# SayanoAI/Comfy-RVC

Hardware: AMD Instinct MI355X
Metric: audio-sec/wall-sec (xRT), 40k_v2 end-to-end VC (higher is better)
Workload: dtype f32; 1 GPU; Full VC 40k_v2 (HuBERT -> RMVPE -> SynthesizerTrnMs768NSFsid), 30 s 16 kHz clips, 12 per GPU per step (3 in flight), vc_single host array in -> int16 host array out (BASELINE.json configs[2]); clips_in_flight_per_gpu=3, weights=procedural (comfy-rvc_amd/synthetic.py), noise=device generator, seeded per clip, parallelism=clip-per-GPU x1 (3 lanes each), one RCCL gather of the step's int16 waveforms

## Files before the change

### comfy-rvc_amd/_lib.py

```python
import ctypes as C
import os

_HERE = os.path.dirname(os.path.abspath(__file__))
LIB_PATH = os.environ.get("RVC_HIP_LIB") or os.path.join(_HERE, "csrc", "librvc_hip.so")


class RvcHipError(RuntimeError):
    pass


def _load():
    if not os.path.isfile(LIB_PATH):
        raise RvcHipError(
            f"{LIB_PATH} is missing: build it with `python -c 'import __graft_entry__ as g; g.build()'` "
            "(or `make -C comfy-rvc_amd/csrc`).  There is no CPU fallback.")
    return C.CDLL(LIB_PATH)


lib = _load()

c_void_p, c_int, c_int64, c_float, c_char_p = C.c_void_p, C.c_int, C.c_int64, C.c_float, C.c_char_p
P = C.POINTER


# ... 177 lines not shown
    "rvc_segment_energy": (c_int, [c_void_p, c_void_p, c_int64, c_int, c_void_p]),
    "rvc_spectrogram_batch": (c_int, [c_void_p, c_void_p, c_void_p, c_int64, c_void_p, c_int, c_int, c_int, c_float, c_int, c_void_p, c_int64]),
    "rvc_mel_filterbank_set": (c_int, [c_void_p, c_int, c_int, c_void_p, c_void_p, c_void_p]),
    "rvc_spec_to_mel_batch": (c_int, [c_void_p, c_void_p, c_void_p, c_int64, c_void_p, c_int, c_int, c_int, c_void_p, c_int64]),
    "rvc_spectrogram_batch_ms": (c_int, [c_void_p, c_void_p, c_void_p, c_int64, c_void_p, c_int, c_int, c_int, c_float, c_int, c_void_p, c_int64]),
    "rvc_mel_spectrogram_vjp": (c_int, [c_void_p, c_void_p, c_void_p, c_int64, c_void_p, c_int, c_int, c_int, c_float, c_int, c_int, c_void_p, c_int64,
                                        c_void_p]),
    "rvc_mel_spectrogram_vjp_launch_count": (c_int, []),
    "rvc_mel_loss_cotangents": (c_int, [c_void_p, c_int, P(c_void_p), P(c_void_p), P(c_int64), c_int, c_float, c_float, P(c_float), P(c_void_p)]),
    "rvc_multiscale_mel_loss": (c_int, [c_void_p, c_void_p, c_int, P(c_void_p), P(c_int64), P(c_int64), c_int, c_int64, P(C.c_int32), P(C.c_int32), c_int, c_int,
                                        c_void_p]),
    "rvc_hpss": (c_int, [c_void_p, c_void_p, c_int, c_int, c_int, c_void_p, c_void_p, c_int]),
    "rvc_hpss_l1": (c_int, [c_void_p, c_void_p, c_void_p, c_int, c_int, c_int, c_float, c_void_p]),
    "rvc_tsi_terms": (c_int, [c_void_p, c_void_p, c_void_p, c_int, c_int, c_int, c_float, c_void_p]),
    "rvc_op_gemm_split": (c_int, [c_void_p] * 7 + [c_int] * 4 + [c_float, c_int, c_float] + [c_int] * 5),
    "rvc_op_conv2d_split": (c_int, [c_void_p] * 7 + [c_int] * 9),
    "rvc_op_wn_in_gate_split": (c_int, [c_void_p] * 6 + [c_int] * 4),
    "rvc_op_gemm_split_qkv": (c_int, [c_void_p] * 6 + [c_int] * 4),
    "rvc_op_conv1d_s2_split": (c_int, [c_void_p] * 6 + [c_int] * 5),
    "rvc_op_conv1d_split": (c_int, [c_void_p] * 6 + [c_int] * 9),
    "rvc_op_conv1d": (c_int, [c_void_p, c_void_p, c_void_p, c_void_p, c_void_p, c_void_p] + [c_int] * 8 +
                      [c_int, c_float, c_int, c_float, c_int, c_float, c_int]),
    "rvc_op_conv_transpose1d": (c_int, [c_void_p, c_void_p, c_void_p, c_void_p, c_void_p] + [c_int] * 6 + [c_int, c_float, c_int]),
    "rvc_op_conv2d3x3": (c_int, [c_void_p, c_void_p, c_void_p, c_void_p, c_void_p, c_void_p] + [c_int] * 5),
    "rvc_op_conv_transpose2d": (c_int, [c_void_p, c_void_p, c_void_p, c_void_p, c_void_p] + [c_int] * 5),
    "rvc_op_gemm_tn": (c_int, [c_void_p, c_void_p, c_void_p, c_void_p] + [c_int] * 4),
    "rvc_conv1d_plan_create": (c_int, [c_void_p, c_void_p] + [c_int] * 7 + [P(c_void_p)]),
    "rvc_conv1d_plan_run": (c_int, [c_void_p, c_void_p, c_void_p, c_int, c_void_p, c_void_p, c_int, c_float, c_int, c_float]),
    "rvc_conv1d_plan_pair_run": (c_int, [c_void_p, c_void_p, c_void_p, c_void_p, c_int, c_void_p, c_float, c_int]),
    "rvc_conv1d_plan_resblock_run": (c_int, [P(c_void_p), c_void_p, c_void_p, c_int, c_void_p, c_float, c_int, P(c_int), c_void_p, c_void_p, c_void_p]),
    "rvc_conv1d_plan_pair_split_run": (c_int, [c_void_p, c_void_p, c_void_p, c_void_p, c_int, c_void_p, c_float, c_int]),
    "rvc_conv1d_plan_destroy": (c_int, [c_void_p]),
    "rvc_op_attention": (c_int, [c_void_p, c_void_p, c_void_p, c_void_p, c_void_p, c_void_p, c_int, c_int]),
    "rvc_op_attention_split": (c_int, [c_void_p] * 7 + [c_int, c_int]),
    "rvc_op_attention_split_rel": (c_int, [c_void_p] * 9 + [c_int, c_int, c_int]),
    "rvc_op_cbr2_small": (c_int, [c_void_p] * 7 + [c_int, c_int, c_int]),
    "rvc_op_layernorm_c_split": (c_int, [c_void_p] * 6 + [c_int, c_int]),
    "rvc_op_conv3_small": (c_int, [c_void_p] * 7 + [c_int] * 6),
    "rvc_op_gemm_split_swapped": (c_int, [c_void_p] * 4 + [c_int] * 5),
    "rvc_op_conv2d3x3_plus_1x1": (c_int, [c_void_p] * 7 + [c_int] * 6),
    "rvc_op_gemm_split_swapped_res": (c_int, [c_void_p] * 5 + [c_int] * 5),
    "rvc_op_attention_rel": (c_int, [c_void_p] * 8 + [c_int, c_int, c_void_p, c_void_p]),
    "rvc_op_layernorm_c": (c_int, [c_void_p] * 6 + [c_int, c_int]),
    "rvc_resample": (c_int, [c_void_p, c_void_p, c_int64, c_void_p, c_int, c_int, c_int, c_void_p, c_int64]),
    "rvc_set_conv_precision": (c_int, [c_int]),
    "rvc_set_pair_arithmetic": (c_int, [c_int]),
# ... 112 lines not shown
```

### comfy-rvc_amd/csrc/conv_kernels.h

```cpp
#pragma once
#include "rvc_internal.h"
#include <hip/hip_ext.h>

namespace rvc {

typedef float f32x16 __attribute__((ext_vector_type(16)));
typedef unsigned int u32x4 __attribute__((ext_vector_type(4)));

struct ConvArgsX : ConvArgs {
  long long ldW;
  int Wcols;
  int Wrows;
  int ksplit; float* partial; long long ldP;
  unsigned magRP, magPW;
  int ni; unsigned magNI;
  const unsigned char* Wx; int CoPx; int xbufs; int NC; int kreal; long long wxBatch;
  const unsigned char* Wx2; const float* bias1; int fuse_p2; float fuse_slope;
  const unsigned char* Xs; long long xsTp;
  unsigned char* Ys; long long ysTp; float ys_slope;
  int wbufs;
  int xcd_remap;
  int h2;
};

// ... 126 lines not shown
bool conv_x3g_plan(ConvPlan& p);
bool conv_x3pf_plan(ConvPlan& p);
bool conv_rbh_plan(ConvPlan& p);
bool conv_x3_pair_plan(const ConvLayer& c1, const ConvLayer& c2, const float* X, long long ldX, int T, long long Tplan, float* Y, long long ldY,
                       const ConvEpilogue& e2, int h2, ConvPlan& p);

struct Rb3Args {
  const float* X; long long ldX; float* Y; long long ldY;
  const unsigned char* W[6];
  const float* B[6];
  int CoPx;
  int T, halo, NO;
  float pre_slope, mid_slope, out_scale;
  const float* nsrc; const float* nw; const float* nb;
};
struct Rb3Plan {
  Rb3Args a; void (*launch)(const Rb3Args&, dim3, size_t, hipStream_t) = nullptr; dim3 grid; size_t lds = 0;
  int C = 0, k = 0, accumulate = 0;
};
bool conv_rb3_plan(const ConvLayer* const* c1, const ConvLayer* const* c2, const float* X, long long ldX, int T, long long Tplan, float* Y, long long ldY,
                   float pre_slope, float out_scale, int accumulate, int h2, const float* nsrc, const float* nw, const float* nb, Rb3Plan& p);
void conv_rb3_launch(const Rb3Plan& p, hipStream_t s);

}
```

### comfy-rvc_amd/csrc/conv_mfma.hip

```cpp
#include "conv_kernels.h"
#include "phase_timing.h"
#include <atomic>
#include <tuple>

#ifndef RVC_EPI_TWOPHASE
#define RVC_EPI_TWOPHASE 0
#endif

namespace rvc {

RVC_PHASE_TABLE_REGISTER;

constexpr int kWSlots = 32;
__host__ __device__ constexpr int x_slots(int BN, int MODE) {
  return MODE == 2 ? (BN >= 512 ? 26 : (BN >= 256 ? 18 : 14)) : (BN >= 512 ? 36 : (BN >= 256 ? 20 : (BN >= 128 ? 32 : 16)));
}

template <int WM, int WN, int AM, int AN, int MODE>
__global__ __launch_bounds__(256) void conv_mfma_kernel(const ConvArgsX p) {
  constexpr int BM = WM * AM * 32, BN = WN * AN * 32;
  constexpr int XS = x_slots(BN, MODE);
  extern __shared__ __attribute__((aligned(16))) float smem[];
  const int CK = p.CK, WROW = p.WROW;
  float* Xs = smem;
// ... 525 lines not shown
  L.nchunk = (Ci + L.CK - 1) / L.CK;
  L.wBatch = (long long)L.nchunk * L.ktaps * L.CK * L.CoP;
  std::vector<float> P((size_t)L.wBatch, 0.f);
  for (int r = 0; r < u; ++r)
    for (int co = 0; co < Co; ++co)
      for (int ci = 0; ci < Ci; ++ci)
        for (int j = 0; j < L.ktaps; ++j) {
          const int e = E2 - j;
          const int kk = e * u + r + pad;
          if (kk < 0 || kk >= k) continue;
          const int chunk = ci / L.CK, vcc = ci % L.CK;
          P[(((size_t)chunk * L.ktaps + j) * L.CK + vcc) * L.CoP + (size_t)co * u + r] = w[((size_t)ci * Co + co) * k + kk];
        }
  if ((g_precision == 2 || (g_precision == 1 && g_x3_default)) && Ci % 16 == 0 && L.Co >= 32) {
    std::vector<float> Weq((size_t)L.Co * Ci * L.ktaps, 0.f);
    for (int r = 0; r < u; ++r)
      for (int co = 0; co < Co; ++co)
        for (int ci = 0; ci < Ci; ++ci)
          for (int j = 0; j < L.ktaps; ++j) {
            const int kk = (E2 - j) * u + r + pad;
            if (kk >= 0 && kk < k) Weq[(((size_t)co * u + r) * Ci + ci) * L.ktaps + j] = w[((size_t)ci * Co + co) * k + kk];
          }
    pack_x3(L, Weq.data(), L.Co, Ci, L.ktaps);
  }
  L.k = k; L.pad = pad;
  L.dil = 1;
  L.conv_pad = E2;
  upload_layer(L, P, bias, Co);
}

void conv2d_kx_layer_init(ConvLayer& L, const float* w, const float* bias, int Co, int Ci, int KH, int KW, int PH, int PWL) {
  RVC_REQUIRE(Ci % 16 == 0 && KH >= 1 && KW >= 1 && PH >= 0 && PH < KH && PWL >= 0 && PWL < KW, "conv2d_kx: Ci must be a multiple of 16, padding inside the window");
  L.mode = 2; L.groups = 1; L.Ci = Ci; L.Co = Co; L.co_real = Co; L.CoP = (Co + 31) & ~31;
  L.k = KH * KW; L.stride = 1; L.dil = 1; L.pad = 0; L.tconv_u = 0; L.up2 = 0; L.ktaps = KH * KW;
  L.kh = KH; L.kw = KW; L.ph = PH; L.pwl = PWL;
  L.CK = 16; L.nchunk = Ci / 16; L.wBatch = 0;
  pack_x3(L, w, Co, Ci, KH * KW);
  L.bd_ = bias ? dev_upload(bias, Co) : nullptr;
}
void conv2d3x3_layer_init(ConvLayer& L, const float* w, const float* bias, int Co, int Ci) {
  L.mode = 2; L.groups = 1; L.Ci = Ci; L.Co = Co; L.co_real = Co; L.CoP = (Co + 31) & ~31;
  L.k = 3; L.stride = 1; L.dil = 1; L.pad = 1; L.tconv_u = 0; L.up2 = 0; L.ktaps = 9;
  L.CK = pick_ck(Ci, 9, 1);
  L.nchunk = (Ci + L.CK - 1) / L.CK;
  L.wBatch = (long long)L.nchunk * 9 * L.CK * L.CoP;
  std::vector<float> P((size_t)L.wBatch, 0.f);
// ... 132 lines not shown
  pe.armed = false;
  if (pe.launches == 1) {
    (void)hipEventDestroy(t.a); (void)hipEventDestroy(t.b);
    t.a = pe.ka; t.b = pe.kb;
  } else {
    (void)hipEventDestroy(pe.ka); (void)hipEventDestroy(pe.kb);
  }
  pe.ka = pe.kb = nullptr;
  ProfRec r{t.a, t.b, flops, cfg, bytes, 0, 0, 0, 0, 0, 0, 0, 1, fused, blocks, 0};
  if (a) { r.h2 = a->h2; r.Ci = a->Ci; r.Co = a->Co; r.k = a->kreal > 0 ? a->kreal : a->ktaps; r.dil = a->dil; r.stride = a->stride; r.Tout = a->Tout; r.Wd = a->Wd; r.ksplit = a->ksplit > 0 ? a->ksplit : 1; }
  std::lock_guard<std::mutex> lk(g_prof_mu);
  g_prof.push_back(r);
}
int conv_prof_dump_csv(const char* path) {
  std::lock_guard<std::mutex> lk(g_prof_mu);
  FILE* f = fopen(path, "w");
  if (!f) return -1;
  fprintf(f, "launch,kernel,tile,Ci,Co,k,dil,stride,Tout,Wd,fused_pair,ksplit,workgroups,us,alg_gflop,alg_mbytes,tflops,alg_gbps,mfma_per_product\n");
  int i = 0;
  for (auto& r : g_prof) {
    (void)hipEventSynchronize(r.b);
    float t = 0.f;
    if (hipEventElapsedTime(&t, r.a, r.b) != hipSuccess) continue;
    static const char* kX3Fam[8] = {"conv_x3_kernel", "conv_x3p_kernel", "conv_x3g_kernel", "conv_x3pf_kernel", "conv_x3s_kernel", "conv_rbh_kernel", "conv_x3q_kernel", "conv_rb3_kernel"};
    fprintf(f, "%d,%s,%s,%d,%d,%d,%d,%d,%d,%d,%d,%d,%lld,%.2f,%.4f,%.3f,%.2f,%.1f,%d\n", i++, r.cfg >= 14 ? kX3Fam[(r.fused >> 4) & 7] : "conv_mfma_kernel", kCfgNames[r.cfg],
            r.Ci, r.Co, r.k, r.dil, r.stride, r.Tout, r.Wd, r.fused & 15, r.ksplit, r.blocks, t * 1e3, r.flops / 1e9, r.bytes / 1e6,
            t > 0 ? r.flops / t / 1e9 : 0.0, t > 0 ? r.bytes / t / 1e6 : 0.0, r.cfg >= 14 ? (r.h2 ? 2 : 3) : 1);
  }
  fclose(f);
  return i;
}
double conv_alg_bytes(const ConvArgsX& a, int batch) {
  const double in = (double)a.Ci * (a.Wd > 0 ? (double)a.Tin * a.Wd : (double)a.Tin);
  const double out = (double)a.Co * a.Tout;
  const double w = (double)a.Co * a.Ci * (a.kreal > 0 ? a.kreal : a.ktaps);
  const bool r_is_x = a.R != nullptr && a.R == a.X;
  return 4.0 * (batch * (in + out * (1.0 + ((a.R && !r_is_x) ? 1.0 : 0.0) + (a.accumulate ? 1.0 : 0.0))) + w);
}
int conv_prof_collect_ex(double* out, double ridge_fp32, double ridge_x3) {
  std::lock_guard<std::mutex> lk(g_prof_mu);
  for (int i = 0; i < kProfCfgs * 8; ++i) out[i] = 0;
  for (auto& r : g_prof) {
    (void)hipEventSynchronize(r.b);
    float t = 0.f;
    if (hipEventElapsedTime(&t, r.a, r.b) != hipSuccess) continue;
    const double ridge = r.cfg >= 14 ? ridge_x3 : ridge_fp32;
    const int o = (r.bytes > 0 && r.flops / r.bytes < ridge) ? 4 : 0;
    double* q = out + r.cfg * 8 + o;
// ... 135 lines not shown
  if (e.tout_limit > 0 && e.tout_limit < Tout) { RVC_REQUIRE(L.tconv_u == 0, "tout_limit on a transposed conv"); Tout = e.tout_limit; }
  auto gemm_cols = [&](int tout) { return L.tconv_u > 0 ? (tout + L.tconv_u - 1) / L.tconv_u : tout; };
  a.Tout = gemm_cols(Tout);
  RVC_REQUIRE(e.plan_tin == 0 || (e.plan_tin >= Tin && !e.tout_limit), "plan_tin is the input length of the whole sequence this launch is a column window of");
  const long long Tplan = e.plan_tin > 0 ? gemm_cols(conv1d_out_len(L, e.plan_tin)) : a.Tout;
  if (L.tconv_u > 0) {
    a.pad = L.conv_pad;
    a.ostride = L.tconv_u; a.orows = L.co_real;
    RVC_REQUIRE(ldY == Tout, "interleaved ConvTranspose1d store needs a dense output (ldY == Tout)");
    RVC_REQUIRE(e.R == nullptr, "residual not supported on the interleaved store");
  } else {
    a.pad = L.pad; a.ostride = 1; a.orows = L.Co;
  }
  a.xBatch = (long long)L.Ci * ldX; a.wBatch = L.wBatch; a.yBatch = (long long)L.Co * ldY; a.rBatch = (long long)L.Co * e.ldR;
  a.bBatch = L.Co;
  const double flops = L.tconv_u > 0 ? 2.0 * Tin * L.Ci * L.co_real * L.k
                                     : 2.0 * L.groups * (double)L.Co * a.Tout * L.Ci * L.k;
  a.Wx = reinterpret_cast<const unsigned char*>(L.Wx_); a.CoPx = L.CoPx; a.wxBatch = L.wxBatch; a.kreal = L.tconv_u > 0 ? L.ktaps : L.k;
  if (e.h2) {
    RVC_REQUIRE(L.Wh_ && (e.xs_in || e.ys_out), "fp16x2 arithmetic is for the two halves of a split-resident ResBlock pair (conv1d_pair_h2_eligible)");
    a.Wx = reinterpret_cast<const unsigned char*>(L.Wh_); a.h2 = 1;
  }
  ConvPlan p;
  if (L.Wx_ && conv_x3_plan(a, L.groups, Tplan, p)) { p.flops = flops; conv_plan_launch(p, s); }
  else {
    RVC_REQUIRE(!e.xs_in && !e.ys_out, "split-resident tensors need the bf16x3 kernel (check conv1d_split_eligible first)");
    run_conv(a, 1, L.groups, Tplan, s, flops);
  }
  if (post) {
    RVC_REQUIRE(L.tconv_u == 0, "post-activation on a transposed conv");
    act_res_inplace(s, Y, e0.R, L.groups * L.Co, Tout, ldY, e0.ldR, e0.act, e0.act_slope, e0.act_before_res);
  }
}

bool conv1d_pair_h2_eligible(const ConvLayer& c1, const ConvLayer& c2, int Tin, int h2) {
  if (!h2 || !c1.Wh_ || !c2.Wh_) return false;
  return conv1d_split_eligible(c1, Tin, SPLIT_PRODUCER, 1) && conv1d_split_eligible(c2, Tin, SPLIT_CONSUMER, 1);
}

static bool plan_split_role(const ConvLayer& L, int Tin, SplitRole role, int h2, ConvPlan& p) {
  if (L.mode != 1 || !L.Wx_ || (h2 && !L.Wh_) || L.tconv_u || L.stride != 1 || L.groups != 1 || (L.Co & 31) || (L.Ci & 15)) return false;
  if (conv1d_out_len(L, Tin) != Tin || L.pad > kSplitMargin) return false;
  ConvArgsX a{};
  a.Ci = L.Ci; a.Co = L.Co; a.CoP = L.CoP; a.Tin = Tin; a.Wd = 0; a.ktaps = L.ktaps; a.dil = L.dil; a.stride = 1; a.pad = L.pad;
  a.Tout = conv1d_out_len(L, Tin); a.ostride = 1; a.orows = L.Co; a.ldX = Tin; a.ldY = a.Tout; a.ldR = a.Tout;
  a.Wx = reinterpret_cast<const unsigned char*>(L.Wx_); a.CoPx = L.CoPx; a.kreal = L.k; a.h2 = h2;
  if (role == SPLIT_CONSUMER) a.R = reinterpret_cast<const float*>(L.Wx_);
// ... 63 lines not shown
```

### comfy-rvc_amd/csrc/rvc_api.hip

```cpp
#include "models.h"
#include "conv_kernels.h"

namespace rvc {
static thread_local std::string g_err;
void set_error(const std::string& msg) { g_err = msg; }
}

using namespace rvc;

struct rvc_ctx { Ctx c; };
static std::mutex g_ctx_mu;
static std::map<int, int> g_ctx_count;
struct rvc_hubert { Hubert* m; rvc_ctx* ctx; };
struct rvc_rmvpe { Rmvpe* m; rvc_ctx* ctx; };
struct rvc_synth { Synth* m; rvc_ctx* ctx; };
struct rvc_conv1d_plan { OwnedConvLayer L; };

#define RVC_TRY try {
#define RVC_CATCH                                                            \
  return 0;                                                                  \
  }                                                                          \
  catch (const std::exception& e) { rvc::set_error(e.what()); return 1; }    \
  catch (...) { rvc::set_error("unknown error"); return 2; }

// ... 1290 lines not shown
  xs.alloc(ib); RVC_HIP_CHECK(hipMemsetAsync(xs.p, 0, ib, s));
  yp.alloc((size_t)Co * T);
  pad2d_split(s, x, (long long)H * W, Ci, H, W, nullptr, 0, xs.p, tp, g.margin);
  ConvEpilogue e; e.act = act; e.act_slope = 0.1f; e.act_before_res = act_before_res;
  if (res) { rp.alloc((size_t)Co * T); pad2d_split(s, res, (long long)H * W, Co, H, W, rp.p, T, nullptr, 0, 0); e.R = rp.p; e.ldR = T; }
  if (ysplit_f32) { ys.alloc(ob); RVC_HIP_CHECK(hipMemsetAsync(ys.p, 0, ob, s)); e.ys_out = ys.p; e.ys_tp = tp; }
  { X3sForceScope force(ksplit, am, an); conv_x3s_run(L, s, xs.p, tp, T, yp.p, T, e, &g); }
  unpad2d(s, yp.p, T, Co, H, W, y, (long long)H * W);
  if (ysplit_f32) {
    RVC_REQUIRE((Co & 15) == 0, "split output needs Co % 16 == 0");
    t.alloc((size_t)Co * T);
    split_image_to_f32(s, ys.p + (size_t)(g.margin - kSplitMargin) * 16, tp, Co, T, t.p, T);
    unpad2d(s, t.p, T, Co, H, W, ysplit_f32, (long long)H * W);
  }
  check_launch();
  RVC_HIP_CHECK(hipStreamSynchronize(s));
  RVC_CATCH
}
int rvc_op_conv_transpose1d(void* stream, const float* x, const float* w, const float* bias, float* y, int Ci, int Co, int Tin, int k, int u,
                            int pad, int pre_act, float pre_slope, int accumulate) {
  RVC_TRY
  OwnedConvLayer L;
  tconv1d_layer_init(L, w, bias, Ci, Co, k, u, pad);
  ConvEpilogue e; e.pre_act = pre_act; e.pre_slope = pre_slope; e.accumulate = accumulate;
  const int Tout = conv1d_out_len(L, Tin);
  conv1d_run(L, (hipStream_t)stream, x, Tin, Tin, y, Tout, e);
  check_launch();
  RVC_HIP_CHECK(hipStreamSynchronize((hipStream_t)stream));
  RVC_CATCH
}
int rvc_op_conv2d3x3(void* stream, const float* x, const float* w, const float* bias, const float* res, float* y, int Ci, int Co, int H, int W,
                     int relu) {
  RVC_TRY
  OwnedConvLayer L;
  conv2d3x3_layer_init(L, w, bias, Co, Ci);
  ConvEpilogue e; e.act = relu ? ACT_RELU : ACT_NONE; e.act_before_res = 1; e.R = res; e.ldR = (long long)H * W;
  conv2d_run(L, (hipStream_t)stream, x, (long long)H * W, H, W, y, (long long)H * W, e);
  check_launch();
  RVC_HIP_CHECK(hipStreamSynchronize((hipStream_t)stream));
  RVC_CATCH
}
int rvc_op_conv_transpose2d(void* stream, const float* x, const float* w, const float* bias, float* y, int Ci, int Co, int H, int W, int relu) {
  RVC_TRY
  OwnedConvLayer L;
  tconv2d_layer_init(L, w, bias, Ci, Co);
  ConvEpilogue e; e.act = relu ? ACT_RELU : ACT_NONE;
  conv2d_run(L, (hipStream_t)stream, x, (long long)H * W, H, W, y, 4LL * H * W, e);
  check_launch();
  RVC_HIP_CHECK(hipStreamSynchronize((hipStream_t)stream));
// ... 380 lines not shown
```

### comfy-rvc_amd/csrc/rvc_internal.h

```cpp
#pragma once
#include <atomic>
#include <hip/hip_runtime.h>
#include <cstdint>
#include <cstdio>
#include <cstdlib>
#include <cmath>
#include <cstring>
#include <map>
#include <mutex>
#include <string>
#include <vector>
#include <stdexcept>

namespace rvc {

void set_error(const std::string& msg);
struct Error : std::runtime_error { using std::runtime_error::runtime_error; };

#define RVC_HIP_CHECK(expr)                                                                       \
  do {                                                                                            \
    hipError_t _e = (expr);                                                                       \
    if (_e != hipSuccess)                                                                         \
      throw rvc::Error(std::string(#expr) + " failed: " + hipGetErrorString(_e) + " (" + __FILE__ + \
                       ":" + std::to_string(__LINE__) + ")");                                     \
// ... 38 lines not shown
  float out_scale; int accumulate;
  int ostride, orows;
  int up2;
  int KH, KW, PH, PWL;
};

struct ConvLayer {
  float* Wd_ = nullptr;
  float* bd_ = nullptr;
  float* bd4_ = nullptr;
  int mode = 1;
  int Ci = 0, Co = 0, CoP = 0, groups = 1;
  int k = 1, stride = 1, dil = 1, pad = 0;
  int ktaps = 1, CK = 8, KT = 1, nchunk = 1;
  int tconv_u = 0;
  int co_real = 0;
  int up2 = 0;
  int conv_pad = 0;
  long long wBatch = 0;
  int kh = 3, kw = 3, ph = 1, pwl = 1;
  uint16_t* Wx_ = nullptr;
  int CoPx = 0; long long wxBatch = 0;
  uint16_t* Wh_ = nullptr;
  int seg2_chunks = 0;
};

struct ConvEpilogue {
  const float* R = nullptr; long long ldR = 0;
  int pre_act = ACT_NONE; float pre_slope = 0.f;
  int act = ACT_NONE; float act_slope = 0.f;
  int act_before_res = 0;
  float out_scale = 1.f; int accumulate = 0;
  const float* bias_override = nullptr;
  int tout_limit = 0;
  int plan_tin = 0;
  const unsigned char* xs_in = nullptr; long long xs_tp = 0;
  unsigned char* ys_out = nullptr; long long ys_tp = 0; float ys_slope = 1.f;
  unsigned char* vt_out = nullptr; long long vt_tp = 0; int vt_row0 = 0;
  int gate_h = 0; const float* gate_g = nullptr;
  int ys_deint_h = 0;
  int h2 = 0;
};
constexpr int kSplitMargin = 64;
inline long long split_image_tp(long long T) { return (T + kSplitMargin + 704 + 63) & ~63LL; }
inline size_t split_image_bytes(int C, long long T) { return (size_t)(C / 16) * 2 * (size_t)split_image_tp(T) * 32; }
enum SplitRole : int { SPLIT_CONSUMER = 0, SPLIT_PRODUCER = 1 };
bool conv1d_split_eligible(const ConvLayer& L, int Tin, SplitRole role = SPLIT_CONSUMER, int h2 = 0);
bool conv1d_pair_h2_eligible(const ConvLayer& c1, const ConvLayer& c2, int Tin, int h2);
int conv1d_residual_period(const ConvLayer& L, int Tin, int h2);
int conv_set_pair_arithmetic(int mode);


void conv1d_layer_init(ConvLayer& L, const float* w , const float* bias, int Co, int Ci, int k,
                       int stride, int pad, int dil, int groups);
void tconv1d_layer_init(ConvLayer& L, const float* w , const float* bias, int Ci, int Co, int k, int u, int pad);
void conv2d3x3_layer_init(ConvLayer& L, const float* w , const float* bias, int Co, int Ci);
void conv2d1x1_layer_init(ConvLayer& L, const float* w , const float* bias, int Co, int Ci);
// ... 133 lines not shown

template <typename T> struct DevBuf {
  T* p = nullptr; size_t n = 0;
  DevBuf() = default;
  ~DevBuf() { dev_free(p); }
  DevBuf(DevBuf&& o) noexcept : p(o.p), n(o.n) { o.p = nullptr; o.n = 0; }
  DevBuf& operator=(DevBuf&& o) noexcept { if (this != &o) { dev_free(p); p = o.p; n = o.n; o.p = nullptr; o.n = 0; } return *this; }
  DevBuf(const DevBuf&) = delete; DevBuf& operator=(const DevBuf&) = delete;
  T* get() const { return p; }
  void reset() { dev_free(p); p = nullptr; n = 0; }
  void alloc(size_t cnt) { reset(); p = static_cast<T*>(dev_alloc(cnt * sizeof(T))); n = cnt; }
  void upload(const T* h, size_t cnt) { reset(); p = dev_upload(h, cnt); n = cnt; }
  void upload(const std::vector<T>& h) { upload(h.data(), h.size()); }
};

struct OwnedConvLayer : ConvLayer {
  OwnedConvLayer() = default;
  ~OwnedConvLayer() { free_weights(); }
  OwnedConvLayer(OwnedConvLayer&& o) noexcept : ConvLayer(o) { o.disown(); }
  OwnedConvLayer& operator=(OwnedConvLayer&& o) noexcept { if (this != &o) { free_weights(); ConvLayer::operator=(o); o.disown(); } return *this; }
  OwnedConvLayer(const OwnedConvLayer&) = delete; OwnedConvLayer& operator=(const OwnedConvLayer&) = delete;
  OwnedConvLayer(const ConvLayer&) = delete; OwnedConvLayer& operator=(const ConvLayer&) = delete;
 private:
  void disown() { Wd_ = bd_ = bd4_ = nullptr; Wx_ = Wh_ = nullptr; }
  void free_weights() { dev_free(Wd_); dev_free(bd_); dev_free(bd4_); dev_free(Wx_); dev_free(Wh_); }
};

#define RVC_ALLOW_BIG_LDS(kern)                                                                                                              \
  do {                                                                                                                                       \
    static std::atomic<unsigned long long> rvc_lds_mask_[4];                                                                                 \
    int rvc_dev_ = 0; (void)hipGetDevice(&rvc_dev_);                                                                                         \
    const unsigned long long rvc_bit_ = 1ull << (rvc_dev_ & 63);                                                                             \
    std::atomic<unsigned long long>& rvc_m_ = rvc_lds_mask_[(rvc_dev_ >> 6) & 3];                                                            \
    if (!(rvc_m_.load(std::memory_order_acquire) & rvc_bit_)) {                                                                              \
      RVC_HIP_CHECK(hipFuncSetAttribute(reinterpret_cast<const void*>(kern), hipFuncAttributeMaxDynamicSharedMemorySize, 160 * 1024));      \
      rvc_m_.fetch_or(rvc_bit_, std::memory_order_release);                                                                                  \
    }                                                                                                                                        \
  } while (0)

struct Arena {
  char* base = nullptr; size_t cap = 0, off = 0, peak = 0; bool dry = false;
  unsigned gen = 0;
  void reset() { off = 0; }
  template <typename T> T* alloc(size_t n) {
    size_t bytes = (n * sizeof(T) + 255) & ~size_t(255);
    size_t o = off; off += bytes; if (off > peak) peak = off;
    if (dry) return reinterpret_cast<T*>(uintptr_t(0x1000) + o);
    RVC_REQUIRE(off <= cap, "arena overflow");
// ... 32 lines not shown
```

### include/rvc_hip.h

```cpp
#ifndef RVC_HIP_H
#define RVC_HIP_H
#include <stdint.h>

#ifdef __cplusplus
extern "C" {
#endif

typedef struct rvc_ctx rvc_ctx;
typedef struct rvc_hubert rvc_hubert;
typedef struct rvc_rmvpe rvc_rmvpe;
typedef struct rvc_synth rvc_synth;

const char* rvc_last_error(void);
const char* rvc_version(void);

int rvc_ctx_create(int device_id, rvc_ctx** out);
int rvc_ctx_destroy(rvc_ctx* ctx);
int64_t rvc_ctx_workspace_bytes(rvc_ctx* ctx);
int rvc_ctx_set_conv_precision(rvc_ctx* ctx, int mode);

typedef struct rvc_hubert_taps {
  float* conv_stack;
  float* pos_conv;
  float* hidden_0;
// ... 248 lines not shown
                     int stride, int pad, float slope, int* units_out);
int rvc_op_disc_conv_plan(int S, int Ci, int Co, int H, int p, int k, int stride, int pad, int* info);
int rvc_op_disc_conv_input_grad(void* stream, const float* d_dev, const float* w_host, const float* cot_dev, const float* a_dev, float* y_dev, int S, int Ci, int Co,
                                int H, int Hd, int p, int stride, float slope, int* units_out);
int rvc_op_disc_conv_input_grad_plan(int S, int Ci, int Co, int H, int Hd, int p, int stride, int* info);
int rvc_op_disc_conv_weight_grad(void* stream, const float* d_dev, const float* x_dev, float* dw_dev, int S, int Ci, int Co, int H, int p, int k, int stride, int pad,
                                 int* splits_out);
int rvc_op_disc_conv_weight_grad_plan(int S, int Ci, int Co, int H, int p, int k, int stride, int pad, int* info);
int rvc_op_conv1d_input_grad(void* stream, const float* d_dev, const float* w_host, const float* a_dev, const float* res_dev, float* y_dev, int transposed, int Ci,
                             int Co, int k, int step, int pad, int64_t N, int64_t Td, int64_t ldD, int64_t ldY, float slope, float scale, int accumulate,
                             int* bm_out, int* units_out);
int rvc_op_conv1d_input_grad_plan(int transposed, int Ci, int Co, int k, int step, int pad, int64_t N, int64_t Td, int* info);
int rvc_op_gemm_split(void* stream, const float* x_dev, const float* w_host, const float* bias_host, const float* res_dev, float* y_dev,
                      float* ysplit_f32_dev, int Ci, int Co, int T, int act, float act_slope, int act_before_res, float out_scale, int ksplit,
                      int am, int an, int k, int dil);
int rvc_op_conv1d_split(void* stream, const float* x_dev, const float* w_host, const float* bias_host, const float* res_dev, float* y_dev,
                        int Ci, int Co, int T, int k, int pad, int dil, int groups, int act, int act_before_res);
int rvc_op_conv1d_s2_split(void* stream, const float* x_dev, const float* w_host, const float* bias_host, float* y_dev, float* y_img_f32_dev, int Ci, int Co, int T, int k,
                           int act);
int rvc_op_conv2d_split(void* stream, const float* x_dev, const float* w_host, const float* bias_host, const float* res_dev, float* y_dev,
                        float* ysplit_f32_dev, int Ci, int Co, int H, int W, int act, int act_before_res, int ksplit, int am, int an);
int rvc_op_conv_transpose1d(void* stream, const float* x_dev, const float* w_host, const float* bias_host, float* y_dev, int Ci, int Co,
                            int Tin, int k, int u, int pad, int pre_act, float pre_slope, int accumulate);
int rvc_op_conv2d3x3(void* stream, const float* x_dev, const float* w_host, const float* bias_host, const float* res_dev, float* y_dev,
                     int Ci, int Co, int H, int W, int relu);
int rvc_op_conv_transpose2d(void* stream, const float* x_dev, const float* w_host, const float* bias_host, float* y_dev, int Ci, int Co,
                            int H, int W, int relu);
int rvc_op_gemm_tn(void* stream, const float* a_dev, const float* b_dev, float* y_dev, int M, int N, int K, int batch);
typedef struct rvc_conv1d_plan rvc_conv1d_plan;
int rvc_conv1d_plan_create(const float* w_host, const float* bias_host, int Ci, int Co, int k, int stride, int pad, int dil, int groups,
                           rvc_conv1d_plan** out);
int rvc_conv1d_plan_run(rvc_conv1d_plan* p, void* stream, const float* x_dev, int Tin, const float* res_dev, float* y_dev, int pre_act,
                        float pre_slope, int act, float act_slope);
int rvc_conv1d_plan_pair_split_run(rvc_conv1d_plan* c1, rvc_conv1d_plan* c2, void* stream, const float* x_dev, int T, float* y_dev,
                                   float out_scale, int accumulate);
int rvc_conv1d_plan_pair_run(rvc_conv1d_plan* c1, rvc_conv1d_plan* c2, void* stream, const float* x_dev, int T, float* y_dev, float out_scale,
                             int accumulate);
int rvc_conv1d_plan_resblock_run(rvc_conv1d_plan* const* plans6, void* stream, const float* x_dev, int T, float* y_dev, float out_scale, int accumulate,
                                 int* ran_out, const float* noise_src_dev, const float* noise_w_dev, const float* noise_b_dev);
int rvc_conv1d_plan_pair_arithmetic(rvc_conv1d_plan* c1, rvc_conv1d_plan* c2, int T);
int rvc_conv1d_plan_destroy(rvc_conv1d_plan* p);
int rvc_op_attention(void* stream, const float* q_dev, const float* k_dev, const float* v_rm_dev, const float* bv_dev, float* out_dev,
                     int heads, int T);
int rvc_op_attention_split(void* stream, const float* q_dev, const float* k_dev, const float* v_dev, const float* bv_dev, float* out_dev,
                           float* out_img_f32_dev, int heads, int T);
int rvc_op_attention_split_rel(void* stream, const float* q_dev, const float* k_dev, const float* v_dev, const float* bv_dev, const float* ek_host,
// ... 63 lines not shown
```

Measured before the change: 2477 audio-sec/wall-sec.

## Add polyphase transposed-conv1d MFMA kernel sharing input tiles across upsample phases

Adds a dedicated conv_tup kernel for transposed 1D convolutions with upsample factors 2/10/12. The weights are packed per polyphase unit (bf16 hi/lo split) so that one input tile in LDS feeds all u output phases, and outputs are written interleaved with 8-byte stores. The path replaces the generic x3 kernel when that kernel would take its 'p' variant, or always in the standalone transposed-conv op. It adds extra weight memory and the bf16x3 split keeps f32-like accuracy, but register pressure with U accumulators per block could hurt occupancy.

Result: no change. 2500 audio-sec/wall-sec (median of 6 runs) (+0.9%).

```diff
diff --git a/comfy-rvc_amd/_lib.py b/comfy-rvc_amd/_lib.py
--- a/comfy-rvc_amd/_lib.py
+++ b/comfy-rvc_amd/_lib.py
@@ -223,6 +223,7 @@
     "rvc_op_conv1d": (c_int, [c_void_p, c_void_p, c_void_p, c_void_p, c_void_p, c_void_p] + [c_int] * 8 +
                       [c_int, c_float, c_int, c_float, c_int, c_float, c_int]),
     "rvc_op_conv_transpose1d": (c_int, [c_void_p, c_void_p, c_void_p, c_void_p, c_void_p] + [c_int] * 6 + [c_int, c_float, c_int]),
+    "rvc_op_conv_transpose1d_window": (c_int, [c_void_p, c_void_p, c_void_p, c_void_p, c_void_p] + [c_int] * 7 + [c_int, c_float]),
     "rvc_op_conv2d3x3": (c_int, [c_void_p, c_void_p, c_void_p, c_void_p, c_void_p, c_void_p] + [c_int] * 5),
     "rvc_op_conv_transpose2d": (c_int, [c_void_p, c_void_p, c_void_p, c_void_p, c_void_p] + [c_int] * 5),
     "rvc_op_gemm_tn": (c_int, [c_void_p, c_void_p, c_void_p, c_void_p] + [c_int] * 4),
diff --git a/comfy-rvc_amd/csrc/conv_kernels.h b/comfy-rvc_amd/csrc/conv_kernels.h
--- a/comfy-rvc_amd/csrc/conv_kernels.h
+++ b/comfy-rvc_amd/csrc/conv_kernels.h
@@ -172,4 +172,22 @@
                    float pre_slope, float out_scale, int accumulate, int h2, const float* nsrc, const float* nw, const float* nb, Rb3Plan& p);
 void conv_rb3_launch(const Rb3Plan& p, hipStream_t s);
 
+struct TupArgs {
+  const float* X; long long ldX; float* Y; long long ldY;
+  const unsigned char* Wt; const float* bias;
+  int Ci, co_real, Tin;
+  int ktaps, pad;
+  int nunits; unsigned mask[3];
+  int P;
+  int ngroups, xcd_remap;
+  float pre_slope, lslope, out_scale;
+};
+struct TupPlan {
+  TupArgs a; void (*launch)(const TupArgs&, dim3, size_t, hipStream_t) = nullptr; dim3 grid; size_t lds = 0;
+  ConvArgsX shape;
+  double alg_bytes = 0.0, flops = 0.0;
+};
+bool conv_tup_plan(const ConvLayer& L, const ConvArgsX& a0, long long Tplan, TupPlan& p);
+void conv_tup_launch(const TupPlan& p, hipStream_t s);
+
 }
diff --git a/comfy-rvc_amd/csrc/conv_mfma.hip b/comfy-rvc_amd/csrc/conv_mfma.hip
--- a/comfy-rvc_amd/csrc/conv_mfma.hip
+++ b/comfy-rvc_amd/csrc/conv_mfma.hip
@@ -571,6 +571,34 @@
             if (kk >= 0 && kk < k) Weq[(((size_t)co * u + r) * Ci + ci) * L.ktaps + j] = w[((size_t)ci * Co + co) * k + kk];
           }
     pack_x3(L, Weq.data(), L.Co, Ci, L.ktaps);
+    if (Co % 32 == 0 && L.ktaps <= 3 && u <= 32) {
+      int NU = 0, uidx[3][32];
+      for (int j = 0; j < L.ktaps; ++j) {
+        L.tup_mask[j] = 0;
+        for (int r = 0; r < u; ++r) {
+          const int kk = (E2 - j) * u + r + pad;
+          if (kk >= 0 && kk < k) { L.tup_mask[j] |= 1u << r; uidx[j][r] = NU++; }
+        }
+      }
+      L.tup_units = NU;
+      const int nck = Ci / 16, G = Co / 32;
+      std::vector<uint16_t> P((size_t)G * nck * NU * 1024, 0);
+      for (int j = 0; j < L.ktaps; ++j)
+        for (int r = 0; r < u; ++r) {
+          if (!((L.tup_mask[j] >> r) & 1u)) continue;
+          const int kk = (E2 - j) * u + r + pad;
+          for (int co = 0; co < Co; ++co)
+            for (int ci = 0; ci < Ci; ++ci) {
+              const float v = w[((size_t)ci * Co + co) * k + kk];
+              const uint16_t hi = bf16_rne(v), lo = bf16_rne(v - bf16_to_f32(hi));
+              const int c16 = ci & 15;
+              const size_t at = ((((size_t)(co >> 5) * nck + (ci >> 4)) * NU + uidx[j][r]) * 1024) + ((size_t)(c16 >> 3) * 32 + (co & 31)) * 8 + (c16 & 7);
+              P[at] = hi; P[at + 512] = lo;
+            }
+        }
+      RVC_HIP_CHECK(hipMalloc(&L.Wt_, P.size() * sizeof(uint16_t)));
+      RVC_HIP_CHECK(hipMemcpy(L.Wt_, P.data(), P.size() * sizeof(uint16_t), hipMemcpyHostToDevice));
+    }
   }
   L.k = k; L.pad = pad;
   L.dil = 1;
@@ -749,8 +777,9 @@
     (void)hipEventSynchronize(r.b);
     float t = 0.f;
     if (hipEventElapsedTime(&t, r.a, r.b) != hipSuccess) continue;
-    static const char* kX3Fam[8] = {"conv_x3_kernel", "conv_x3p_kernel", "conv_x3g_kernel", "conv_x3pf_kernel", "conv_x3s_kernel", "conv_rbh_kernel", "conv_x3q_kernel", "conv_rb3_kernel"};
-    fprintf(f, "%d,%s,%s,%d,%d,%d,%d,%d,%d,%d,%d,%d,%lld,%.2f,%.4f,%.3f,%.2f,%.1f,%d\n", i++, r.cfg >= 14 ? kX3Fam[(r.fused >> 4) & 7] : "conv_mfma_kernel", kCfgNames[r.cfg],
+    static const char* kX3Fam[16] = {"conv_x3_kernel", "conv_x3p_kernel", "conv_x3g_kernel", "conv_x3pf_kernel", "conv_x3s_kernel", "conv_rbh_kernel", "conv_x3q_kernel", "conv_rb3_kernel",
+                                     "conv_tup_kernel", "", "", "", "", "", "", ""};
+    fprintf(f, "%d,%s,%s,%d,%d,%d,%d,%d,%d,%d,%d,%d,%lld,%.2f,%.4f,%.3f,%.2f,%.1f,%d\n", i++, r.cfg >= 14 ? kX3Fam[(r.fused >> 4) & 15] : "conv_mfma_kernel", kCfgNames[r.cfg],
             r.Ci, r.Co, r.k, r.dil, r.stride, r.Tout, r.Wd, r.fused & 15, r.ksplit, r.blocks, t * 1e3, r.flops / 1e9, r.bytes / 1e6,
             t > 0 ? r.flops / t / 1e9 : 0.0, t > 0 ? r.bytes / t / 1e6 : 0.0, r.cfg >= 14 ? (r.h2 ? 2 : 3) : 1);
   }
@@ -932,7 +961,11 @@
     a.Wx = reinterpret_cast<const unsigned char*>(L.Wh_); a.h2 = 1;
   }
   ConvPlan p;
-  if (L.Wx_ && conv_x3_plan(a, L.groups, Tplan, p)) { p.flops = flops; conv_plan_launch(p, s); }
+  TupPlan tp;
+  const bool x3 = L.Wx_ && conv_x3_plan(a, L.groups, Tplan, p);
+  const bool x3p = x3 && (p.prof_fused >> 4) == 1;
+  if (L.tconv_u > 0 && (x3p || e.tup_any_len) && conv_tup_plan(L, a, Tplan, tp)) { tp.flops = flops; conv_tup_launch(tp, s); }
+  else if (x3) { p.flops = flops; conv_plan_launch(p, s); }
   else {
     RVC_REQUIRE(!e.xs_in && !e.ys_out, "split-resident tensors need the bf16x3 kernel (check conv1d_split_eligible first)");
     run_conv(a, 1, L.groups, Tplan, s, flops);
diff --git a/comfy-rvc_amd/csrc/conv_tup.hip b/comfy-rvc_amd/csrc/conv_tup.hip
--- /dev/null
+++ b/comfy-rvc_amd/csrc/conv_tup.hip
@@ -0,0 +1,201 @@
+#include "conv_x3_dev.h"
+
+namespace rvc {
+
+template <int U, int NB, int NW>
+__global__ __launch_bounds__(NW * 64) void conv_tup_kernel(const TupArgs p) {
+  constexpr int KTM = 3;
+  constexpr int BN = NW * NB * 32, NT = NW * 64;
+  constexpr int XS = (2 * (BN + KTM - 1) + NT - 1) / NT;
+  static_assert(U % 2 == 0, "8-byte stores");
+  extern __shared__ __attribute__((aligned(1024))) unsigned char smem_tup[];
+  const int P = p.P;
+  const int xhalf = P * 16, xplane = 2 * xhalf, xbuf = 2 * xplane;
+  const int wslot = p.nunits * 2048;
+  unsigned char* Xs = smem_tup;
+  unsigned char* Ws = smem_tup + ((2 * xbuf + 1023) & ~1023);
+
+  const int tid = threadIdx.x, lane = tid & 63;
+  const int wave = __builtin_amdgcn_readfirstlane(tid >> 6);
+  const int li = lane & 31, lh = lane >> 5;
+  const unsigned tile = p.xcd_remap ? xcd_tile(blockIdx.x, gridDim.x) : blockIdx.x;
+  const int tile_x = (int)(tile / (unsigned)p.ngroups), g = (int)(tile - (unsigned)tile_x * (unsigned)p.ngroups);
+  const int n0 = tile_x * BN, bx = n0 - p.pad;
+  const int nck = p.Ci >> 4;
+  const float pre_slope = p.pre_slope;
+  const __amdgpu_buffer_rsrc_t xrs = make_rsrc(p.X, (unsigned)p.Ci * (unsigned)p.ldX * 4u);
+  const __amdgpu_buffer_rsrc_t wrs = make_rsrc(p.Wt + (long long)g * nck * wslot, (unsigned)nck * (unsigned)wslot);
+
+  f32x16 acc[U][NB];
+#pragma unroll
+  for (int r = 0; r < U; ++r)
+#pragma unroll
+    for (int nb = 0; nb < NB; ++nb)
+#pragma unroll
+      for (int i = 0; i < 16; ++i) acc[r][nb][i] = 0.f;
+
+  float xr[XS][8];
+  auto slot_geom = [&](int s, int& hb, int& q) -> bool {
+    const int i = tid + NT * s;
+    hb = i >= P ? 1 : 0;
+    q = i - hb * P;
+    return i < 2 * P;
+  };
+  auto load_slots = [&](int chunk) {
+#pragma unroll
+    for (int s = 0; s < XS; ++s) {
+      int hb, q;
+      const bool ok = slot_geom(s, hb, q);
+      const int x = bx + q;
+      const unsigned voff = (ok && x >= 0 && x < p.Tin) ? ((unsigned)(chunk * 16 + hb * 8) * (unsigned)p.ldX + (unsigned)x) * 4u : kOOB;
+#pragma unroll
+      for (int j = 0; j < 8; ++j) xr[s][j] = buf_load(xrs, voff + (unsigned)j * (unsigned)p.ldX * 4u);
+    }
+  };
+  auto store_slots = [&](int xb) {
+#pragma unroll
+    for (int s = 0; s < XS; ++s) {
+      int hb, q;
+      if (slot_geom(s, hb, q)) {
+        u32x4 hi, lo;
+#pragma unroll
+        for (int j = 0; j < 4; ++j) {
+          const float a = xr[s][2 * j], b = xr[s][2 * j + 1];
+          unsigned h_, l_;
+          split2(fmaxf(a, a * pre_slope), fmaxf(b, b * pre_slope), h_, l_);
+          hi[j] = h_; lo[j] = l_;
+        }
+        unsigned char* d = Xs + xb * xbuf + hb * xhalf + q * 16;
+        *reinterpret_cast<u32x4*>(d) = hi;
+        *reinterpret_cast<u32x4*>(d + xplane) = lo;
+      }
+    }
+  };
+  const int npieces = 2 * p.nunits;
+  auto issue_w = [&](int chunk, int slot) {
+    for (int pi = wave; pi < npieces; pi += NW)
+      buf_dma(wrs, Ws + slot * wslot + pi * 1024, lane * 16, chunk * wslot + pi * 1024);
+  };
+
+  load_slots(0);
+  issue_w(0, 0);
+  wait_vmcnt<0>();
+  store_slots(0);
+
+  const int aoff = lh * 512 + li * 16;
+  const int boff = lh * xhalf + (wave * NB * 32 + li) * 16;
+  for (int c = 0; c < nck; ++c) {
+    const int b = c & 1;
+    lds_barrier();
+    if (c + 1 < nck) { load_slots(c + 1); issue_w(c + 1, b ^ 1); }
+    const unsigned char* wp = Ws + b * wslot + aoff;
+    const unsigned char* xa = Xs + b * xbuf + boff;
+    u32x4 ah = *reinterpret_cast<const u32x4*>(wp), al = *reinterpret_cast<const u32x4*>(wp + 1024);
+    auto tap = [&](auto jc) {
+      constexpr int J = decltype(jc)::value;
+      if (J < p.ktaps) {
+        const unsigned m = p.mask[J];
+        u32x4 bh[NB], bl[NB];
+#pragma unroll
+        for (int nb = 0; nb < NB; ++nb) {
+          bh[nb] = *reinterpret_cast<const u32x4*>(xa + J * 16 + nb * 512);
+          bl[nb] = *reinterpret_cast<const u32x4*>(xa + xplane + J * 16 + nb * 512);
+        }
+        auto phase = [&](auto rc) {
+          constexpr int R = decltype(rc)::value;
+          if ((m >> R) & 1u) {
+            wp += 2048;
+            const u32x4 ahn = *reinterpret_cast<const u32x4*>(wp), aln = *reinterpret_cast<const u32x4*>(wp + 1024);
+#pragma unroll
+            for (int nb = 0; nb < NB; ++nb)
+              acc[R][nb] = __builtin_amdgcn_mfma_f32_32x32x16_bf16(__builtin_bit_cast(bf16x8, ah), __builtin_bit_cast(bf16x8, bl[nb]), acc[R][nb], 0, 0, 0);
+#pragma unroll
+            for (int nb = 0; nb < NB; ++nb)
+              acc[R][nb] = __builtin_amdgcn_mfma_f32_32x32x16_bf16(__builtin_bit_cast(bf16x8, al), __builtin_bit_cast(bf16x8, bh[nb]), acc[R][nb], 0, 0, 0);
+#pragma unroll
+            for (int nb = 0; nb < NB; ++nb)
+              acc[R][nb] = __builtin_amdgcn_mfma_f32_32x32x16_bf16(__builtin_bit_cast(bf16x8, ah), __builtin_bit_cast(bf16x8, bh[nb]), acc[R][nb], 0, 0, 0);
+            ah = ahn; al = aln;
+          }
+        };
+        static_for<0, U>(phase);
+      }
+    };
+    static_for<0, KTM>(tap);
+    if (c + 1 < nck) { wait_vmcnt<0>(); store_slots(b ^ 1); }
+  }
+
+  const __amdgpu_buffer_rsrc_t yrs = make_rsrc(p.Y, (unsigned)p.co_real * (unsigned)p.ldY * 4u);
+  const float lslope = p.lslope, oscale = p.out_scale;
+  typedef unsigned u32x2_t __attribute__((ext_vector_type(2)));
+#pragma unroll
+  for (int nb = 0; nb < NB; ++nb) {
+    const int q = n0 + (wave * NB + nb) * 32 + li;
+#pragma unroll
+    for (int i = 0; i < 16; ++i) {
+      const int co = g * 32 + (i & 3) + 8 * (i >> 2) + 4 * lh;
+      const float bv = p.bias ? p.bias[co] : 0.f;
+      const unsigned off = q < p.Tin ? ((unsigned)co * (unsigned)p.ldY + (unsigned)U * (unsigned)q) * 4u : kOOB;
+#pragma unroll
+      for (int r = 0; r < U; r += 2) {
+        float v0 = acc[r][nb][i] + bv, v1 = acc[r + 1][nb][i] + bv;
+        v0 = fmaxf(v0, v0 * lslope) * oscale; v1 = fmaxf(v1, v1 * lslope) * oscale;
+        __builtin_amdgcn_raw_buffer_store_b64(u32x2_t{__float_as_uint(v0), __float_as_uint(v1)}, yrs, (int)(off + (unsigned)r * 4u), 0, 0);
+      }
+    }
+  }
+}
+
+template <int U, int NB, int NW>
+static void launch_tup(const TupArgs& a, dim3 grid, size_t lds, hipStream_t s) {
+  auto kern = conv_tup_kernel<U, NB, NW>;
+  RVC_ALLOW_BIG_LDS(kern);
+  conv_launch(kern, grid, dim3(NW * 64), lds, s, a);
+}
+
+bool conv_tup_plan(const ConvLayer& L, const ConvArgsX& a0, long long Tplan, TupPlan& p) {
+  const int u = L.tconv_u;
+  if (u <= 0 || !L.Wt_ || L.tup_units <= 0 || L.mode != 1 || L.groups != 1) return false;
+  if ((L.Ci & 15) || (L.co_real & 31) || L.ktaps > 3) return false;
+  if (!(u == 2 || u == 10 || u == 12)) return false;
+  if (a0.R || a0.accumulate || a0.Xs || a0.Ys || a0.h2 || a0.Wd > 0) return false;
+  if (!(a0.act == ACT_NONE || a0.act == ACT_LRELU || a0.act == ACT_RELU) || !(a0.pre_act == ACT_NONE || a0.pre_act == ACT_LRELU)) return false;
+  if (a0.Tout != a0.Tin || a0.ldY != (long long)u * a0.Tin || (reinterpret_cast<uintptr_t>(a0.Y) & 7)) return false;
+  const double Tp = (double)(Tplan > a0.Tin ? Tplan : a0.Tin);
+  if ((double)L.co_real * u * Tp * 4.0 >= 2147483648.0 || (double)L.Ci * (double)a0.ldX * 4.0 >= 2147483648.0 || (double)L.Ci * Tp * 4.0 >= 2147483648.0) return false;
+  const int nck = L.Ci / 16;
+  const long long wslot = (long long)L.tup_units * 2048;
+  if ((double)nck * (double)wslot >= 2147483648.0) return false;
+  const int G = L.co_real / 32;
+  const bool narrow = u != 2 && ((Tplan > a0.Tin ? Tplan : (long long)a0.Tin) + 255) / 256 * G < 256;
+  const int NB = u == 2 ? 2 : 1, NW = (u == 2 || narrow) ? 4 : 8, BN = NW * NB * 32;
+  const int P = BN + L.ktaps - 1;
+  const size_t lds = (size_t)((2 * 2 * P * 32 + 1023) & ~1023) + 2 * (size_t)wslot + 2048;
+  if (lds > 160u * 1024u) return false;
+  p = TupPlan{};
+  TupArgs& a = p.a;
+  a.X = a0.X; a.ldX = a0.ldX; a.Y = a0.Y; a.ldY = a0.ldY;
+  a.Wt = reinterpret_cast<const unsigned char*>(L.Wt_); a.bias = a0.bias;
+  a.Ci = L.Ci; a.co_real = L.co_real; a.Tin = a0.Tin; a.ktaps = L.ktaps; a.pad = L.conv_pad;
+  a.nunits = L.tup_units; a.mask[0] = L.tup_mask[0]; a.mask[1] = L.tup_mask[1]; a.mask[2] = L.tup_mask[2];
+  a.P = P; a.ngroups = G; a.xcd_remap = x3_xcd_remap();
+  a.pre_slope = a0.pre_act == ACT_LRELU ? a0.pre_slope : 1.f;
+  a.lslope = a0.act == ACT_NONE ? 1.f : (a0.act == ACT_RELU ? 0.f : a0.act_slope);
+  a.out_scale = a0.out_scale;
+  p.grid = dim3((unsigned)(((a0.Tin + BN - 1) / BN) * a.ngroups), 1, 1);
+  p.lds = lds;
+  if (u == 2) p.launch = &launch_tup<2, 2, 4>;
+  else if (u == 10) p.launch = narrow ? &launch_tup<10, 1, 4> : &launch_tup<10, 1, 8>;
+  else p.launch = narrow ? &launch_tup<12, 1, 4> : &launch_tup<12, 1, 8>;
+  p.shape = a0; p.shape.kreal = L.k; p.shape.ksplit = 1;
+  p.alg_bytes = 4.0 * ((double)L.Ci * a0.Tin + (double)L.co_real * u * a0.Tin + (double)L.Ci * L.co_real * L.k);
+  return true;
+}
+
+void conv_tup_launch(const TupPlan& p, hipStream_t s) {
+  ProfTicket tk = conv_prof_begin(s);
+  p.launch(p.a, p.grid, p.lds, s);
+  conv_prof_end(tk, s, p.flops, 14 + 8, p.alg_bytes, &p.shape, (long long)p.grid.x, 8 << 4);
+}
+
+}
diff --git a/comfy-rvc_amd/csrc/rvc_api.hip b/comfy-rvc_amd/csrc/rvc_api.hip
--- a/comfy-rvc_amd/csrc/rvc_api.hip
+++ b/comfy-rvc_amd/csrc/rvc_api.hip
@@ -1336,9 +1336,20 @@
   RVC_TRY
   OwnedConvLayer L;
   tconv1d_layer_init(L, w, bias, Ci, Co, k, u, pad);
-  ConvEpilogue e; e.pre_act = pre_act; e.pre_slope = pre_slope; e.accumulate = accumulate;
+  ConvEpilogue e; e.pre_act = pre_act; e.pre_slope = pre_slope; e.accumulate = accumulate; e.tup_any_len = 1;
   const int Tout = conv1d_out_len(L, Tin);
   conv1d_run(L, (hipStream_t)stream, x, Tin, Tin, y, Tout, e);
+  check_launch();
+  RVC_HIP_CHECK(hipStreamSynchronize((hipStream_t)stream));
+  RVC_CATCH
+}
+int rvc_op_conv_transpose1d_window(void* stream, const float* x, const float* w, const float* bias, float* y, int Ci, int Co, int Tin, int plan_tin, int k,
+                                   int u, int pad, int pre_act, float pre_slope) {
+  RVC_TRY
+  OwnedConvLayer L;
+  tconv1d_layer_init(L, w, bias, Ci, Co, k, u, pad);
+  ConvEpilogue e; e.pre_act = pre_act; e.pre_slope = pre_slope; e.plan_tin = plan_tin; e.tup_any_len = 1;
+  conv1d_run(L, (hipStream_t)stream, x, Tin, Tin, y, conv1d_out_len(L, Tin), e);
   check_launch();
   RVC_HIP_CHECK(hipStreamSynchronize((hipStream_t)stream));
   RVC_CATCH
diff --git a/comfy-rvc_amd/csrc/rvc_internal.h b/comfy-rvc_amd/csrc/rvc_internal.h
--- a/comfy-rvc_amd/csrc/rvc_internal.h
+++ b/comfy-rvc_amd/csrc/rvc_internal.h
@@ -84,6 +84,7 @@
   uint16_t* Wx_ = nullptr;
   int CoPx = 0; long long wxBatch = 0;
   uint16_t* Wh_ = nullptr;
+  uint16_t* Wt_ = nullptr; unsigned tup_mask[3] = {0, 0, 0}; int tup_units = 0;
   int seg2_chunks = 0;
 };
 
@@ -95,6 +96,7 @@
   float out_scale = 1.f; int accumulate = 0;
   const float* bias_override = nullptr;
   int tout_limit = 0;
+  int tup_any_len = 0;
   int plan_tin = 0;
   const unsigned char* xs_in = nullptr; long long xs_tp = 0;
   unsigned char* ys_out = nullptr; long long ys_tp = 0; float ys_slope = 1.f;
@@ -274,8 +276,8 @@
   OwnedConvLayer(const OwnedConvLayer&) = delete; OwnedConvLayer& operator=(const OwnedConvLayer&) = delete;
   OwnedConvLayer(const ConvLayer&) = delete; OwnedConvLayer& operator=(const ConvLayer&) = delete;
  private:
-  void disown() { Wd_ = bd_ = bd4_ = nullptr; Wx_ = Wh_ = nullptr; }
-  void free_weights() { dev_free(Wd_); dev_free(bd_); dev_free(bd4_); dev_free(Wx_); dev_free(Wh_); }
+  void disown() { Wd_ = bd_ = bd4_ = nullptr; Wx_ = Wh_ = Wt_ = nullptr; }
+  void free_weights() { dev_free(Wd_); dev_free(bd_); dev_free(bd4_); dev_free(Wx_); dev_free(Wh_); dev_free(Wt_); }
 };
 
 #define RVC_ALLOW_BIG_LDS(kern)                                                                                                              \
diff --git a/include/rvc_hip.h b/include/rvc_hip.h
--- a/include/rvc_hip.h
+++ b/include/rvc_hip.h
@@ -294,6 +294,8 @@
                         float* ysplit_f32_dev, int Ci, int Co, int H, int W, int act, int act_before_res, int ksplit, int am, int an);
 int rvc_op_conv_transpose1d(void* stream, const float* x_dev, const float* w_host, const float* bias_host, float* y_dev, int Ci, int Co,
                             int Tin, int k, int u, int pad, int pre_act, float pre_slope, int accumulate);
+int rvc_op_conv_transpose1d_window(void* stream, const float* x_dev, const float* w_host, const float* bias_host, float* y_dev, int Ci, int Co,
+                                   int Tin, int plan_tin, int k, int u, int pad, int pre_act, float pre_slope);
 int rvc_op_conv2d3x3(void* stream, const float* x_dev, const float* w_host, const float* bias_host, const float* res_dev, float* y_dev,
                      int Ci, int Co, int H, int W, int relu);
 int rvc_op_conv_transpose2d(void* stream, const float* x_dev, const float* w_host, const float* bias_host, float* y_dev, int Ci, int Co,
```
